# gvanhoy/gr-liquiddsp

Measured on AMD Instinct MI355X. Metric: Msamples/s through flex_rx (QPSK r1/2 1024B), higher is better.
Workload: dtype f32; 1 GPU; flex_rx single stream per GPU, 20000000 samples (10 Msym), PSK4 r=1/2 (CONV_V27), 1024-B payload, CRC-24, 256-sample gaps, CFO/phase/delay + AWGN Es/N0=20 dB; frames_decoded_ok=1154, streams_per_gpu=1, blocks_in_flight=12, stage_events=none (fxrx_set_timing level 0), steps=1415, passes=independent captures (reset between passes), segments=256, repairs=0

## Files before the change

gr-liquiddsp_amd/csrc/fx_kernels.hip:

```cpp
#include <hip/hip_runtime.h>
#include <algorithm>
#include "fx_device.h"
#include "fx_launch.h"
#include "fx_vbclean.h"
#include "fx_rsgmd.h"

#define HALF         256

template <int WW> struct WalkLdsT {
    static constexpr int WAVES = WW;
    static constexpr bool SWEEP_PAIRS = WW == 4;
    float2 win[FX_NFFT];
    float2 X[FX_NFFT];
    float2 S[FX_NFFT];
    float2 scr[WW][576];
    float2 v[640];
    float2 P[256];
    float  m2[FX_NFFT];
    float2 hdr[FX_HDR_SYM];
    float2 cw[(WW + 1) * FX_HOP + 8];
    __device__ __forceinline__ float2 *scr2(int wave) { return wave < 2 ? v + 576 * wave : cw + 576 * (wave - 2); }
    float2 pb[16];
    float2 eqw[16];
    float  taps[FX_MF_TAPS];
// ... 1677 lines not shown
#undef FX_CHAIN_LAUNCH
    return hipGetLastError();
}

template <bool SOFT>
__global__ __launch_bounds__(64 * FX_FLEX_WAVES)
void fx_hdrdec_kernel(const uint8_t *in, uint32_t n, uint8_t *out, int32_t *valid, const FxTables *T)
{
    __shared__ WalkLdsT<FX_FLEX_WAVES> L;
    const int tid = threadIdx.x;
    for (uint32_t h = blockIdx.x; h < n; h += gridDim.x) {
        if constexpr (SOFT) { for (int i = tid; i < 8 * FX_HDR_ENC; i += 64 * FX_FLEX_WAVES) L.hsoft()[i] = in[(size_t)h * (8 * FX_HDR_ENC) + i]; }
        else if (tid < FX_HDR_ENC) L.b0[tid] = in[(size_t)h * FX_HDR_ENC + tid];
        __syncthreads();
        if constexpr (SOFT) decode_header_soft(L, T, tid); else decode_header_bytes(L, T, tid);
        if (tid < FX_HDR_DEC) out[(size_t)h * FX_HDR_DEC + tid] = L.b1[tid];
        if (tid == 0) valid[h] = (int32_t)L.u[1];
        __syncthreads();
    }
}
extern "C" hipError_t fx_launch_hdrdec(int soft, unsigned n, hipStream_t st, const uint8_t *in, uint8_t *out, int32_t *valid, const FxTables *T)
{
    if (n == 0) return hipSuccess;
    const unsigned grid = std::min(n, 65536u);
    if (soft) hipLaunchKernelGGL((fx_hdrdec_kernel<true>), dim3(grid), dim3(64 * FX_FLEX_WAVES), 0, st, in, n, out, valid, T);
    else hipLaunchKernelGGL((fx_hdrdec_kernel<false>), dim3(grid), dim3(64 * FX_FLEX_WAVES), 0, st, in, n, out, valid, T);
    return hipGetLastError();
}

#define PLAN_THREADS 256
#define PLAN_NV 7
enum { PV_SYM = 0, PV_BYTE, PV_DW, PV_OUT, PV_MF, PV_JOB, PV_VB };

__device__ __forceinline__ unsigned pll_class(unsigned ms)
{
    switch (ms) {
    case FX_MODEM_PSK2: return 0; case FX_MODEM_PSK4: return 1; case FX_MODEM_PSK8: return 2; case FX_MODEM_PSK16: return 3;
    case FX_MODEM_DPSK2: return 4; case FX_MODEM_DPSK4: return 5; case FX_MODEM_DPSK8: return 6; case FX_MODEM_ASK4: return 7;
    case FX_MODEM_QAM16: return 8; case FX_MODEM_QAM32: return 9; case FX_MODEM_QAM64: return 10; default: return 11;
    }
}

template <int NT> __device__ __forceinline__ void plan_scan(uint32_t (&v)[PLAN_NV], uint32_t (&tot)[PLAN_NV], uint32_t (*ws)[PLAN_NV])
{
    const int tid = threadIdx.x, lane = tid & 63, wave = tid >> 6;
    uint32_t inc[PLAN_NV];
#pragma unroll
    for (int q = 0; q < PLAN_NV; q++) {
        inc[q] = v[q];
#pragma unroll
        for (int d = 1; d < 64; d <<= 1) { const uint32_t o = (uint32_t)__shfl_up((int)inc[q], d, 64); if (lane >= d) inc[q] += o; }
    }
    __syncthreads();
    if (lane == 63) for (int q = 0; q < PLAN_NV; q++) ws[wave][q] = inc[q];
    __syncthreads();
#pragma unroll
    for (int q = 0; q < PLAN_NV; q++) {
        uint32_t wb = 0, t = 0;
#pragma unroll
        for (int w = 0; w < NT / 64; w++) { const uint32_t x = ws[w][q]; if (w < wave) wb += x; t += x; }
        tot[q] = t; v[q] = wb + inc[q] - v[q];
    }
}

#define PLAN_MAXG 256
enum { PW_TICKET = 0, PW_CLS_CNT = 16, PW_DEC_CNT = 28, PW_VBC_CNT = 31, PW_CLS_FILL = 38, PW_DEC_FILL = 50, PW_VBC_FILL = 53,
       PW_FLAG = 128, PW_AGG = 384, PW_INC = 384 + 8 * PLAN_MAXG, PW_WORDS = 384 + 16 * PLAN_MAXG };

__device__ __forceinline__ uint32_t wave_agg_add(uint32_t *counters, uint32_t key, uint32_t inc, bool active)
{
    const int lane = threadIdx.x & 63;
    unsigned long long rem = __ballot(active);
    uint32_t result = 0;
    while (rem) {
        const int leader = __ffsll((long long)rem) - 1;
        const uint32_t k = (uint32_t)__shfl((int)key, leader, 64);
        const bool mine = active && key == k;
        const unsigned long long same = __ballot(mine);
        uint32_t incl = mine ? inc : 0u;
#pragma unroll
        for (int d = 1; d < 64; d <<= 1) { const uint32_t o = (uint32_t)__shfl_up((int)incl, d, 64); if (lane >= d) incl += o; }
        const uint32_t total = (uint32_t)__shfl((int)incl, 63, 64);
        uint32_t base = 0;
        if (lane == leader) base = atomicAdd(&counters[k], total);
        base = (uint32_t)__shfl((int)base, leader, 64);
        if (mine) result = base + incl - inc;
        rem &= ~same;
    }
    return result;
}

struct PlanWords { uint32_t flags, nsym, plen, ms, check, fec0, fec1; };
__device__ __forceinline__ PlanWords plan_words(const FxFrame *fp) { return { fp->flags, fp->pay_sym_len, fp->pay_len, fp->ms, fp->check, fp->fec0, fp->fec1 }; }
struct PlanFrame {
    const FxFrame *fp = nullptr; uint32_t sidx = 0, bps = 0, k = 0, l0 = 0, l1 = 0, nblk = 0, vnb = 0; bool valid = false, batch = false;
};
__device__ __forceinline__ PlanFrame plan_sizes(const PlanWords &w, bool live, uint32_t detect, uint32_t vb_blk, uint32_t (&v)[PLAN_NV])
{
    PlanFrame f;
#pragma unroll
    for (int q = 0; q < PLAN_NV; q++) v[q] = 0u;
    f.valid = live && !detect && (w.flags & FX_FLAG_HEADER_VALID);
    if (!f.valid) return f;
    f.bps = modem_bps(w.ms);
    f.k = w.plen + crc_len(w.check); f.l0 = fec_enc_len(w.fec0, f.k); f.l1 = fec_enc_len(w.fec1, f.l0);
    f.nblk = (w.nsym + 1023u) / 1024u;
    v[PV_SYM] = (w.nsym + 7u) & ~7u;
    v[PV_BYTE] = (max(f.l1, f.k) + 8u + 15u) & ~15u;
    v[PV_DW] = ((8u * max(f.l0, f.k) + 6u + 63u) & ~63u) + 64u;
    v[PV_OUT] = (w.plen + 15u) & ~15u;
    v[PV_MF] = f.nblk; v[PV_JOB] = 1u;
    f.batch = vb_blk && conv_p(w.fec0) && !conv_p(w.fec1) && w.fec1 != FX_FEC_RS_M8;
    if (f.batch) { f.vnb = (8u * f.k + 6u + vb_blk - 1u) / vb_blk; v[PV_VB] = f.vnb; }
    return f;
}
__device__ __forceinline__ bool plan_demote(uint32_t vb_before, uint32_t vnb, uint32_t vb_cap) { return (uint64_t)vb_before + vnb + 7u * 128u > vb_cap; }

struct PlanKey {
    uint32_t cls, rs, vc;
    __device__ uint32_t dec(bool batch) const { return batch ? 2u : rs; }
    __device__ uint32_t pack() const { return cls | rs << 4 | vc << 5; }
    __device__ static PlanKey unpack(uint32_t p) { return { p & 15u, (p >> 4) & 1u, (p >> 5) & 7u }; }
};
__device__ __forceinline__ PlanKey plan_key(uint32_t ms, uint32_t fec0, uint32_t fec1)
{
    const uint32_t p = (uint32_t)conv_p(fec0);
    return { pll_class(ms), (fec0 == FX_FEC_RS_M8 || fec1 == FX_FEC_RS_M8) ? 1u : 0u, p ? p - 1u : 0u };
}

__device__ __forceinline__ uint32_t plan_stream_of(const uint32_t *base, uint32_t nstreams, uint32_t g)
{
    uint32_t lo = 0, hi = nstreams;
    while (hi - lo > 1) { const uint32_t mid = (lo + hi) >> 1; if (base[mid] <= g) lo = mid; else hi = mid; }
    return lo;
}

struct PlanRest {
    const float2 *x, *xa_end; int64_t abs_base;
    int64_t start; int32_t offset; float rxy, tau, gamma, dphi, phi; uint32_t pfb; int32_t mfc0; uint32_t mix_th, mix_dl; float mf_scale;
    float pilot_dphi, pilot_phi, pilot_gain; uint32_t pll_th; float pll_f; uint32_t header[FX_HDR_DEC / 4];
};
__device__ __forceinline__ PlanRest plan_rest(const FxFrame *__restrict__ fp, const FxStreamDesc *__restrict__ sd)
{
    PlanRest r;
    r.x = sd->x; r.xa_end = sd->xa_end; r.abs_base = sd->abs_base;
    r.start = fp->start; r.offset = fp->offset; r.rxy = fp->rxy; r.tau = fp->tau; r.gamma = fp->gamma; r.dphi = fp->dphi; r.phi = fp->phi;
    r.pfb = fp->pfb; r.mfc0 = fp->mfc0; r.mix_th = fp->mix_th; r.mix_dl = fp->mix_dl; r.mf_scale = fp->mf_scale;
    r.pilot_dphi = fp->pilot_dphi; r.pilot_phi = fp->pilot_phi; r.pilot_gain = fp->pilot_gain; r.pll_th = fp->pll_th; r.pll_f = fp->pll_f;
    const uint32_t *hw = reinterpret_cast<const uint32_t *>(fp->header);
#pragma unroll
    for (int i = 0; i < FX_HDR_DEC / 4; i++) r.header[i] = hw[i];
    return r;
}
__device__ __forceinline__ void plan_emit(FxPayJob *__restrict__ job, FxOutRec *__restrict__ rec, const PlanRest &fp,
                                          const PlanWords &w, const PlanFrame &f, const uint32_t (&off)[PLAN_NV], uint32_t eq, uint32_t slot, uint32_t vb_off)
{
    FxPayJob j;
    j.x = fp.x; j.xa_end = fp.xa_end; j.start = fp.start; j.mix_th = fp.mix_th; j.mix_dl = fp.mix_dl; j.mf_scale = fp.mf_scale;
    j.pfb = fp.pfb; j.mfc0 = fp.mfc0; j.pll_th = fp.pll_th; j.pll_f = fp.pll_f; j.ms = w.ms; j.bps = f.bps;
    j.nsym = f.valid ? w.nsym : 0u; j.sym_off = off[PV_SYM];
    j.pay_len = w.plen; j.check = w.check; j.fec0 = w.fec0; j.fec1 = w.fec1; j.k = f.k; j.l0 = f.l0; j.l1 = f.l1;
    j.byte_off = off[PV_BYTE]; j.dw_off = off[PV_DW]; j.out_off = off[PV_OUT]; j.pad_ = f.valid ? 1u : 0u;
    j.eq = eq; j.chain_idx = slot; j.vb_off = vb_off; j.vb_nblk = (uint16_t)f.vnb; j.vb_clean = 0;
    *job = j;
    union { FxOutRec r; uint4 q[sizeof(FxOutRec) / 16]; } u;
    u.r.start = fp.abs_base + fp.start; u.r.stream = f.sidx; u.r.offset = fp.offset;
    u.r.rxy = fp.rxy; u.r.tau = fp.tau; u.r.gamma = fp.gamma; u.r.dphi = fp.dphi; u.r.phi = fp.phi; u.r.pfb = fp.pfb;
    u.r.pilot_dphi = fp.pilot_dphi; u.r.pilot_phi = fp.pilot_phi; u.r.pilot_gain = fp.pilot_gain;
    u.r.flags = w.flags & FX_FLAG_HEADER_VALID;
    u.r.pay_len = f.valid ? w.plen : 0u; u.r.ms = w.ms; u.r.check = w.check; u.r.fec0 = w.fec0; u.r.fec1 = w.fec1;
    u.r.nsym = f.valid ? w.nsym : 0u; u.r.bps = f.bps; u.r.sym_off = off[PV_SYM]; u.r.out_off = off[PV_OUT];
    u.r.evm_sum = 0.0f; u.r.payload_valid = 0; u.r.status = 0;
    uint32_t *rw = reinterpret_cast<uint32_t *>(u.r.header);
#pragma unroll
    for (int i = 0; i < FX_HDR_DEC / 4; i++) rw[i] = fp.header[i];
    u.r.byte_off = off[PV_BYTE];
    uint4 *dst = reinterpret_cast<uint4 *>(rec);
#pragma unroll
    for (int i = 0; i < (int)(sizeof(FxOutRec) / 16); i++) dst[i] = u.q[i];
}

template <bool AGENT> struct PlanCounts {
    const uint32_t *cls_, *dec_, *vbc_;
    __device__ __forceinline__ static uint32_t ld(const uint32_t *p)
    {
        if constexpr (AGENT) return __hip_atomic_load(p, __ATOMIC_RELAXED, __HIP_MEMORY_SCOPE_AGENT); else return *p;
    }
    __device__ __forceinline__ uint32_t cls(int c) const { return ld(cls_ + c); }
    __device__ __forceinline__ uint32_t dec(int c) const { return ld(dec_ + c); }
    __device__ __forceinline__ uint32_t vbc(int c) const { return ld(vbc_ + c); }
};
template <class Counts> __device__ __forceinline__ void plan_class_bases(const Counts &cnt, uint32_t (&cls_base)[FX_PLL_CLASSES + 1], uint32_t (&vbc_base)[8])
{
    uint32_t b = 0;
    for (int c = 0; c < FX_PLL_CLASSES; c++) { cls_base[c] = b; b += (cnt.cls(c) + 63u) & ~63u; }
    cls_base[FX_PLL_CLASSES] = b;
    uint32_t vb = 0;
    for (int c = 0; c < 7; c++) { vbc_base[c] = vb; vb += (cnt.vbc(c) + 127u) & ~127u; }
    vbc_base[7] = vb;
}
template <int NT, class Counts> __device__ __forceinline__ void plan_pad_lists(const Counts &cnt, const uint32_t (&cls_base)[FX_PLL_CLASSES + 1], const uint32_t (&vbc_base)[8], const FxPlanArgs &a)
{
    for (int c = 0; c < FX_PLL_CLASSES; c++)
        for (uint32_t i = cls_base[c] + cnt.cls(c) + threadIdx.x; i < cls_base[c + 1] && i < a.list_cap; i += NT) a.pll_list[i] = 0xFFFFFFFFu;
    for (int c = 0; c < 7; c++)
        for (uint32_t i = vbc_base[c] + cnt.vbc(c) + threadIdx.x; i < vbc_base[c + 1] && i < a.vb_cap; i += NT) a.vb_items[i] = 0xFFFFFFFFu;
}
template <class Tot, class Counts> __device__ __forceinline__ void plan_fill_hdr(FxBlockHdr &h, uint32_t N, Tot tot, const Counts &cnt, const uint32_t (&cls_base)[FX_PLL_CLASSES + 1],
                                                                                 const uint32_t (&vbc_base)[8], const FxPlanArgs &a)
{
    h.n_frames = N; h.n_pjobs = tot[PV_JOB]; h.n_mfblk = min(tot[PV_MF], a.mf_cap);
    h.n_dec_plain = cnt.dec(0); h.n_dec_rs = cnt.dec(1); h.n_dec_batch = cnt.dec(2);
    h.n_vb_items = min(vbc_base[7], a.vb_cap); h.vb_blk = a.vb_blk; h.vb_want = tot[PV_VB] + 7u * 128u; h.n_vb_fallback = 0;
    for (int c = 0; c < FX_PLL_CLASSES; c++) { h.pll_cnt[c] = cnt.cls(c); h.pll_base[c] = cls_base[c]; }
    h.pll_base[FX_PLL_CLASSES] = cls_base[FX_PLL_CLASSES];
    h.sym_total = tot[PV_SYM]; h.byte_total = tot[PV_BYTE]; h.dw_total = tot[PV_DW]; h.out_total = tot[PV_OUT];
    h.done = 1;
}
template <int NT> __device__ __forceinline__ void plan_mirror_hdr(const FxBlockHdr &h, const FxPlanArgs &a)
{
    const uint32_t *src = reinterpret_cast<const uint32_t *>(&h);
    uint32_t *d0 = reinterpret_cast<uint32_t *>(a.hdr_pay), *d1 = reinterpret_cast<uint32_t *>(a.hdr_host), *z = reinterpret_cast<uint32_t *>(a.hdr);
    for (int i = threadIdx.x; i < (int)(sizeof(FxBlockHdr) / 4); i += NT) { const uint32_t w = src[i]; d0[i] = w; d1[i] = w; z[i] = 0u; }
}

__device__ __forceinline__ PlanFrame plan_frame(uint32_t g, bool live, const FxPlanArgs &a, PlanWords &w, uint32_t (&v)[PLAN_NV])
{
    const uint32_t sidx = live ? plan_stream_of(a.stream_base, a.nstreams, g) : 0u;
    const FxFrame *fp = live ? a.chain + a.streams[sidx].chain_base + (g - a.stream_base[sidx]) : nullptr;
    w = live ? plan_words(fp) : PlanWords{};
    PlanFrame f = plan_sizes(w, live, a.detect, a.vb_blk, v);
    f.fp = fp; f.sidx = sidx;
    return f;
}
__device__ __forceinline__ void plan_range(uint32_t N, uint32_t &g0, uint32_t &g1)
{
    const uint32_t per = ((N + gridDim.x - 1) / gridDim.x + PLAN_THREADS - 1) / PLAN_THREADS * PLAN_THREADS;
    g0 = min(N, blockIdx.x * per); g1 = min(N, g0 + per);
}
template <int NT> __device__ __forceinline__ uint32_t plan_stream_bases(const uint32_t *chain_count, uint32_t nstreams, uint32_t *stream_base, uint32_t (*ws)[PLAN_NV])
{
    const int tid = threadIdx.x;
    uint32_t run = 0;
    for (uint32_t s0 = 0; s0 < nstreams; s0 += NT) {
        const uint32_t sidx = s0 + tid;
        uint32_t v[PLAN_NV] = { sidx < nstreams ? chain_count[sidx] : 0u, 0, 0, 0, 0, 0, 0 }, tot[PLAN_NV];
        plan_scan<NT>(v, tot, ws);
        if (sidx < nstreams) stream_base[sidx] = run + v[0];
        run += tot[0];
        __syncthreads();
    }
    if (tid == 0) stream_base[nstreams] = run;
    __threadfence(); __syncthreads(); __threadfence();
    return run;
}

extern "C" __global__ __launch_bounds__(PLAN_THREADS)
void fx_plan_kernel(const FxPlanArgs a)
{
    __shared__ uint32_t ws[PLAN_THREADS / 64][PLAN_NV];
    __shared__ uint32_t base_s[PLAN_NV];
    uint32_t *const pw = a.ws;
    const int tid = threadIdx.x;
    const uint32_t N = plan_stream_bases<PLAN_THREADS>(a.chain_count, a.nstreams, a.stream_base, ws);
    uint32_t g0, g1; plan_range(N, g0, g1);
    const uint32_t wg = blockIdx.x;
    uint32_t run[PLAN_NV] = { 0, 0, 0, 0, 0, 0, 0 };
    for (uint32_t c0 = g0; c0 < g1; c0 += PLAN_THREADS) {
        uint32_t v[PLAN_NV], tot[PLAN_NV]; PlanWords w;
        (void)plan_frame(c0 + tid, c0 + tid < g1, a, w, v);
        plan_scan<PLAN_THREADS>(v, tot, ws);
#pragma unroll
        for (int q = 0; q < PLAN_NV; q++) run[q] += tot[q];
        __syncthreads();
    }
    if (tid == 0) {
        uint32_t base[PLAN_NV] = { 0, 0, 0, 0, 0, 0, 0 };
        if (wg > 0) {
            for (int q = 0; q < PLAN_NV; q++) pw[PW_AGG + 8 * wg + q] = run[q];
            __threadfence();
            __hip_atomic_store(&pw[PW_FLAG + wg], 1u, __ATOMIC_RELEASE, __HIP_MEMORY_SCOPE_AGENT);
            for (int p = (int)wg - 1; p >= 0; p--) {
                uint32_t f;
                do { f = __hip_atomic_load(&pw[PW_FLAG + p], __ATOMIC_ACQUIRE, __HIP_MEMORY_SCOPE_AGENT); if (!f) __builtin_amdgcn_s_sleep(2); } while (!f);
                const volatile uint32_t *src = pw + (f == 2u ? PW_INC : PW_AGG) + 8 * p;
                for (int q = 0; q < PLAN_NV; q++) base[q] += src[q];
                if (f == 2u) break;
            }
        }
        for (int q = 0; q < PLAN_NV; q++) { pw[PW_INC + 8 * wg + q] = base[q] + run[q]; base_s[q] = base[q]; }
        __threadfence();
        __hip_atomic_store(&pw[PW_FLAG + wg], 2u, __ATOMIC_RELEASE, __HIP_MEMORY_SCOPE_AGENT);
    }
    __syncthreads();
    uint32_t before[PLAN_NV];
#pragma unroll
    for (int q = 0; q < PLAN_NV; q++) before[q] = base_s[q];
    for (uint32_t c0 = g0; c0 < g1; c0 += PLAN_THREADS) {
        const uint32_t g = c0 + tid;
        const bool live = g < g1;
        uint32_t v[PLAN_NV], tot[PLAN_NV]; PlanWords w;
        PlanFrame f = plan_frame(g, live, a, w, v);
        plan_scan<PLAN_THREADS>(v, tot, ws);
#pragma unroll
        for (int q = 0; q < PLAN_NV; q++) { v[q] += before[q]; before[q] += tot[q]; }
        if (f.batch && plan_demote(v[PV_VB], f.vnb, a.vb_cap)) { f.batch = false; f.vnb = 0; }
        if (live) {
            plan_emit(a.pjobs + g, a.recs + g, plan_rest(f.fp, a.streams + f.sidx), w, f, v, a.eq, (uint32_t)(f.fp - a.chain), 0u);
            for (uint32_t c = 0; c < f.nblk; c++) if (v[PV_MF] + c < a.mf_cap) { a.mf_job[v[PV_MF] + c] = g; a.mf_c0[v[PV_MF] + c] = c * 1024u; }
        }
        {
            const PlanKey key = plan_key(w.ms, w.fec0, w.fec1);
            (void)wave_agg_add(pw + PW_CLS_CNT, key.cls, 1u, f.valid);
            (void)wave_agg_add(pw + PW_DEC_CNT, key.dec(f.batch), 1u, f.valid);
            (void)wave_agg_add(pw + PW_VBC_CNT, key.vc, f.vnb, f.batch);
        }
        __syncthreads();
    }
}

extern "C" __global__ __launch_bounds__(PLAN_THREADS)
void fx_planlists_kernel(const FxPlanArgs a)
{
    __shared__ struct { FxBlockHdr h; uint32_t cls_base[FX_PLL_CLASSES + 1], vbc_base[8], last; } sh;
    uint32_t *const pw = a.ws;
    const PlanCounts<true> cnt{ pw + PW_CLS_CNT, pw + PW_DEC_CNT, pw + PW_VBC_CNT };
    const int tid = threadIdx.x;
    const uint32_t N = __hip_atomic_load(&a.stream_base[a.nstreams], __ATOMIC_RELAXED, __HIP_MEMORY_SCOPE_AGENT);
    if (tid == 0) plan_class_bases(cnt, sh.cls_base, sh.vbc_base);
    __syncthreads();
    uint32_t g0, g1; plan_range(N, g0, g1);
    for (uint32_t c0 = g0; c0 < g1; c0 += PLAN_THREADS) {
        const uint32_t g = c0 + tid;
        const bool live = g < g1;
        uint32_t ms = 0, fec0 = 0, fec1 = 0, vnb = 0; bool val = false;
        if (live) { const FxPayJob &j = a.pjobs[g]; val = j.pad_ != 0; ms = j.ms; fec0 = j.fec0; fec1 = j.fec1; vnb = j.vb_nblk; }
        const PlanKey key = plan_key(ms, fec0, fec1);
        const bool bt = val && vnb;
        const uint32_t pp = sh.cls_base[key.cls] + wave_agg_add(pw + PW_CLS_FILL, key.cls, 1u, val);
        if (val && pp < a.list_cap) a.pll_list[pp] = g;
        const uint32_t rs = key.dec(bt), dp = wave_agg_add(pw + PW_DEC_FILL, rs, 1u, val);
        if (val && dp < a.list_cap) a.dec_list[(size_t)rs * a.list_cap + dp] = g;
        const uint32_t at = sh.vbc_base[key.vc] + wave_agg_add(pw + PW_VBC_FILL, key.vc, vnb, bt);
        if (bt) a.pjobs[g].vb_off = at;
    }
    if (blockIdx.x == 0) plan_pad_lists<PLAN_THREADS>(cnt, sh.cls_base, sh.vbc_base, a);
    __threadfence(); __syncthreads();
    if (tid == 0) sh.last = atomicAdd(&pw[PW_TICKET], 1u) == gridDim.x - 1 ? 1u : 0u;
    __syncthreads();
    if (!sh.last) return;
    __threadfence();
    if (tid == 0) {
        sh.h = *a.hdr;
        plan_fill_hdr(sh.h, N, (const volatile uint32_t *)(pw + PW_INC + 8 * (gridDim.x - 1)), cnt, sh.cls_base, sh.vbc_base, a);
    }
    __syncthreads();
    plan_mirror_hdr<PLAN_THREADS>(sh.h, a);
    for (int i = tid; i < PW_WORDS; i += PLAN_THREADS) pw[i] = 0u;
}

#define PLAN_TILE 2048
#define PLAN_BATCH 2
#define PLAN_LDS_STREAMS 256
enum { PO_CLS = 0, PO_DEC = FX_PLL_CLASSES, PO_VBC = FX_PLL_CLASSES + 4, PO_N = FX_PLL_CLASSES + 12 };
template <int NT> struct PlanOneShared {
    FxBlockHdr h;
    uint32_t ws[NT / 64][PLAN_NV];
    uint32_t cnt[PO_N], fill[PO_N];
    uint32_t cls_base[FX_PLL_CLASSES + 1], vbc_base[8];
    uint32_t sbase[PLAN_LDS_STREAMS + 1], cbase[PLAN_LDS_STREAMS];
};
template <int NT> __device__ __forceinline__ uint32_t plan_one_slot(uint32_t g, const FxPlanArgs &a, const PlanOneShared<NT> &sh, uint32_t &sidx)
{
    if (a.nstreams <= PLAN_LDS_STREAMS) { sidx = plan_stream_of(sh.sbase, a.nstreams, g); return sh.cbase[sidx] + (g - sh.sbase[sidx]); }
    sidx = plan_stream_of(a.stream_base, a.nstreams, g);
    return a.streams[sidx].chain_base + (g - a.stream_base[sidx]);
}

template <int NT> __global__ __launch_bounds__(NT)
void fx_planfused_kernel(const FxPlanArgs a)
{
    constexpr uint32_t TILE = PLAN_TILE;
    constexpr int KEEP = PLAN_TILE / NT, JB = PLAN_BATCH;
    static_assert(NT % 64 == 0 && KEEP * NT == PLAN_TILE && KEEP % JB == 0, "whole waves; the tile is KEEP frames a thread, in whole batches");
    __shared__ PlanOneShared<NT> sh;
    __shared__ uint2 keep[PLAN_TILE];
    const PlanCounts<false> cnt{ sh.cnt + PO_CLS, sh.cnt + PO_DEC, sh.cnt + PO_VBC };
    const uint32_t tid = threadIdx.x, nstreams = a.nstreams;
#ifdef FX_STAMPS
    unsigned long long tk_ = __builtin_readcyclecounter(); uint32_t st1_ = 0, st2_ = 0, st6_ = 0, st7_ = 0;
#define PLAN_TICK(acc) do { const unsigned long long t_ = __builtin_readcyclecounter(); acc += (uint32_t)(t_ - tk_); tk_ = t_; } while (0)
#else
#define PLAN_TICK(acc) do { } while (0)
#endif
    {
        const uint32_t *src = reinterpret_cast<const uint32_t *>(a.hdr); uint32_t *dst = reinterpret_cast<uint32_t *>(&sh.h);
        for (int i = (int)tid; i < (int)(sizeof(FxBlockHdr) / 4); i += NT) dst[i] = src[i];
        if (tid < PO_N) { sh.cnt[tid] = 0u; sh.fill[tid] = 0u; }
        if (tid <= FX_PLL_CLASSES) sh.cls_base[tid] = 0u;
        if (tid < 8) sh.vbc_base[tid] = 0u;
    }
    uint32_t N;
    if (nstreams <= PLAN_LDS_STREAMS) {
        uint32_t v[PLAN_NV] = { tid < nstreams ? a.chain_count[tid] : 0u, 0, 0, 0, 0, 0, 0 }, tot[PLAN_NV];
        if (nstreams > 1) plan_scan<NT>(v, tot, sh.ws); else { tot[0] = v[0]; v[0] = 0u; }
        if (tid < nstreams) { sh.sbase[tid] = v[0]; a.stream_base[tid] = v[0]; sh.cbase[tid] = a.streams[tid].chain_base; }
        if (tid == 0) { sh.sbase[nstreams] = tot[0]; a.stream_base[nstreams] = tot[0]; }
        __syncthreads();
        N = sh.sbase[nstreams];
    } else N = plan_stream_bases<NT>(a.chain_count, nstreams, a.stream_base, sh.ws);

    uint32_t run[PLAN_NV] = { 0, 0, 0, 0, 0, 0, 0 };
    for (int pass = N > TILE ? 0 : 1; pass < 2; pass++) {
#pragma unroll
        for (int q = 0; q < PLAN_NV; q++) run[q] = 0u;
        for (uint32_t t0 = 0; t0 < N; t0 += TILE) {
            const uint32_t nt = min(TILE, N - t0), t1 = t0 + nt, per = (nt + NT - 1) / NT, f0 = t0 + tid * per;
            uint32_t st[PLAN_NV];
            PlanWords w[KEEP]; uint32_t slot[KEEP], sidx[KEEP];
#pragma unroll
            for (int i = 0; i < KEEP; i++) {
                const bool live = (uint32_t)i < per && f0 + i < t1;
                slot[i] = plan_one_slot(live ? f0 + i : t0, a, sh, sidx[i]);
                w[i] = plan_words(a.chain + slot[i]);
            }
#pragma unroll
            for (int q = 0; q < PLAN_NV; q++) st[q] = 0u;
#pragma unroll
            for (int i = 0; i < KEEP; i++) {
                uint32_t v[PLAN_NV];
                (void)plan_sizes(w[i], (uint32_t)i < per && f0 + i < t1, a.detect, a.vb_blk, v);
#pragma unroll
                for (int q = 0; q < PLAN_NV; q++) st[q] += v[q];
            }
            {
                uint32_t tot[PLAN_NV];
                plan_scan<NT>(st, tot, sh.ws);
#pragma unroll
                for (int q = 0; q < PLAN_NV; q++) { st[q] += run[q]; run[q] += tot[q]; }
            }
            if (pass == 0 || N <= TILE) {
                uint32_t vb = st[PV_VB];
#pragma unroll
                for (int i = 0; i < KEEP; i++) {
                    uint32_t v[PLAN_NV];
                    const PlanFrame f = plan_sizes(w[i], (uint32_t)i < per && f0 + i < t1, a.detect, a.vb_blk, v);
                    const bool batch = f.batch && !plan_demote(vb, f.vnb, a.vb_cap);
                    vb += f.vnb;
                    if (f.valid) {
                        const PlanKey key = plan_key(w[i].ms, w[i].fec0, w[i].fec1);
                        atomicAdd(&sh.cnt[PO_CLS + key.cls], 1u);
                        atomicAdd(&sh.cnt[PO_DEC + key.dec(batch)], 1u);
                        if (batch) atomicAdd(&sh.cnt[PO_VBC + key.vc], f.vnb);
                    }
                }
            }
            if (pass == 0) continue;
            if (t0 == 0) {
                __syncthreads();
                if (tid == 0) plan_class_bases(cnt, sh.cls_base, sh.vbc_base);
                __syncthreads();
            }
            PLAN_TICK(st1_);
#pragma unroll
            for (int b0 = 0; b0 < KEEP; b0 += JB) {
                if ((uint32_t)b0 >= per) break;
                PlanRest r[JB];
#pragma unroll
                for (int i = 0; i < JB; i++) r[i] = plan_rest(a.chain + slot[b0 + i], a.streams + sidx[b0 + i]);
#pragma unroll
                for (int i = 0; i < JB; i++) {
                    const uint32_t g = f0 + b0 + i;
                    if ((uint32_t)(b0 + i) >= per || g >= t1) break;
                    const PlanWords &wi = w[b0 + i];
                    uint32_t v[PLAN_NV];
                    PlanFrame f = plan_sizes(wi, true, a.detect, a.vb_blk, v);
                    f.fp = a.chain + slot[b0 + i]; f.sidx = sidx[b0 + i];
                    if (f.batch && plan_demote(st[PV_VB], f.vnb, a.vb_cap)) { f.batch = false; f.vnb = 0; }
                    uint32_t at = 0;
                    if (f.valid) {
                        const PlanKey key = plan_key(wi.ms, wi.fec0, wi.fec1);
                        const uint32_t pp = sh.cls_base[key.cls] + atomicAdd(&sh.fill[PO_CLS + key.cls], 1u);
                        if (pp < a.list_cap) a.pll_list[pp] = g;
                        const uint32_t rs = key.dec(f.batch), dp = atomicAdd(&sh.fill[PO_DEC + rs], 1u);
                        if (dp < a.list_cap) a.dec_list[(size_t)rs * a.list_cap + dp] = g;
                        if (f.batch) at = sh.vbc_base[key.vc] + atomicAdd(&sh.fill[PO_VBC + key.vc], f.vnb);
                    }
                    keep[g - t0] = make_uint2(st[PV_MF], f.nblk);
                    plan_emit(a.pjobs + g, a.recs + g, r[i], wi, f, st, a.eq, slot[b0 + i], at);
#pragma unroll
                    for (int q = 0; q < PLAN_NV; q++) st[q] += v[q];
                }
            }
            __syncthreads();
            PLAN_TICK(st2_);
            for (uint32_t k = tid >> 4; k < nt; k += NT / 16) {
                const uint2 kp = keep[k];
                const uint32_t g = t0 + k, sub = tid & 15u;
                for (uint32_t c = sub; c < kp.y; c += 16u) if (kp.x + c < a.mf_cap) { a.mf_job[kp.x + c] = g; a.mf_c0[kp.x + c] = c * 1024u; }
            }
            __syncthreads();
        }
    }
    plan_pad_lists<NT>(cnt, sh.cls_base, sh.vbc_base, a);
    PLAN_TICK(st6_);
    __threadfence(); __syncthreads();
    PLAN_TICK(st7_);
    if (tid == 0) {
#ifdef FX_STAMPS
        sh.h.stamp[1] = st1_; sh.h.stamp[2] = st2_; sh.h.stamp[6] = st6_; sh.h.stamp[7] = st7_;
#endif
        plan_fill_hdr(sh.h, N, run, cnt, sh.cls_base, sh.vbc_base, a);
    }
    __syncthreads();
    plan_mirror_hdr<NT>(sh.h, a);
}

extern "C" hipError_t fx_launch_plan(hipStream_t st, unsigned grid, int fused, unsigned threads, const FxPlanArgs &a)
{
    const unsigned g = grid < 1u ? 1u : (grid > PLAN_MAXG ? PLAN_MAXG : grid);
    if (fused && g == 1u) {
        if (threads == 512u) hipLaunchKernelGGL((fx_planfused_kernel<512>), dim3(1), dim3(512), 0, st, a);
        else if (threads == 256u) hipLaunchKernelGGL((fx_planfused_kernel<256>), dim3(1), dim3(256), 0, st, a);
        else return hipErrorInvalidValue;
    } else {
        hipLaunchKernelGGL(fx_plan_kernel, dim3(g), dim3(PLAN_THREADS), 0, st, a);
        hipLaunchKernelGGL(fx_planlists_kernel, dim3(g), dim3(PLAN_THREADS), 0, st, a);
    }
    return hipGetLastError();
}
extern "C" unsigned fx_plan_ws_words(void) { return PW_WORDS; }

#define PMF_THREADS 256
#define PMF_SYMS    1024
#define PMF_SPAN    (2 * PMF_SYMS + FX_MF_TAPS)

__global__ __launch_bounds__(PMF_THREADS)
void fx_paymf_kernel(const FxPayJob *jobs, const uint32_t *blk_job, const uint32_t *blk_c0, const FxBlockHdr *hdr, const FxFrame *chain, float2 *sym_raw,
                     const FxTables *T)
{
    constexpr int LEAD = FX_EQ_TAPS - 1;
    __shared__ float2 v[PMF_SPAN + LEAD + 4];
    __shared__ float2 u[2 * PMF_SYMS + FX_EQ_TAPS];
    __shared__ float2 eqw[16];
    __shared__ float taps[FX_MF_TAPS];
    const uint32_t nitems = hdr->n_mfblk;
    const int tid = threadIdx.x;
    const float2 *sc = T->sc;
    for (uint32_t bi = blockIdx.x; bi < nitems; bi += gridDim.x) {
        const FxPayJob job = jobs[blk_job[bi]];
        const uint32_t c0 = blk_c0[bi];
        const uint32_t ns = min((uint32_t)PMF_SYMS, job.nsym - c0);
        const int64_t sym0 = (int64_t)FX_SYM0_PAY + FX_EQ_DELAY;
        const int64_t nlo = sym_sample(sym0 + c0, job.mfc0) - LEAD - (FX_MF_TAPS - 1);
        const int64_t nhi = sym_sample(sym0 + c0 + ns - 1, job.mfc0);
        const int span = (int)(nhi - nlo + 1);
        const XSrc xs = make_xsrc(job.x, job.xa_end, 0);
        __syncthreads();
        if (tid < FX_MF_TAPS) taps[tid] = T->proto[job.pfb + FX_NPFB * tid];
        if (tid < 16) eqw[tid] = tid < FX_EQ_TAPS ? chain[job.chain_idx].eq[tid] : make_float2(0.0f, 0.0f);
        for (int m = tid; m < span; m += PMF_THREADS) {
            const int64_t nn = nlo + m;
            v[m] = derot(xld(xs, job.start + nn), job.mix_th + job.mix_dl * (uint32_t)nn, sc);
        }
        __syncthreads();
        const int nu = span - (FX_MF_TAPS - 1);
        for (int m = tid; m < nu; m += PMF_THREADS) {
            const float2 y = mf_sum<7>(v, taps, m + (FX_MF_TAPS - 1));
            u[m] = make_float2(y.x * job.mf_scale, y.y * job.mf_scale);
        }
        __syncthreads();
        for (uint32_t i = tid; i < ns; i += PMF_THREADS) {
            const int nc = (int)(sym_sample(sym0 + c0 + i, job.mfc0) - nlo) - (FX_MF_TAPS - 1);
            sym_raw[(size_t)job.sym_off + c0 + i] = eq_sum16(u + nc - (FX_EQ_TAPS - 1), eqw);
        }
    }
}

#define PMF4_STRIDE 274
extern "C" __global__ __launch_bounds__(PMF_THREADS)
void fx_paymf4_kernel(const FxPayJob *jobs, const uint32_t *blk_job, const uint32_t *blk_c0, const FxBlockHdr *hdr, float2 *sym_raw, const FxTables *T)
{
    __shared__ float2 ph[8 * PMF4_STRIDE];
    __shared__ __attribute__((aligned(16))) float taps[FX_MF_TAPS];
    static_assert(FX_MF_TAPS == 28 && PMF_SYMS == 4 * PMF_THREADS, "tile below: 28 taps, four symbols per thread");
    static_assert(PMF4_STRIDE >= (PMF_SPAN + 8) / 8 + 5, "phase arrays hold the span plus the slack phantom symbols read");
    const uint32_t nitems = hdr->n_mfblk;
    const int tid = threadIdx.x;
    const float2 *sc = T->sc;
    for (uint32_t bi = blockIdx.x; bi < nitems; bi += gridDim.x) {
        const FxPayJob job = jobs[blk_job[bi]];
        const uint32_t c0 = blk_c0[bi];
        const uint32_t ns = min((uint32_t)PMF_SYMS, job.nsym - c0);
        const int64_t nlo = sym_sample((int64_t)FX_SYM0_PAY + c0, job.mfc0) - (FX_MF_TAPS - 1);
        const int span = 2 * (int)ns + (FX_MF_TAPS - 2);
        const float2 *px = job.x, *pa = job.xa_end;
        const int64_t p0 = job.start + nlo;
        const uint32_t th0 = job.mix_th + job.mix_dl * (uint32_t)nlo, dl = job.mix_dl;
        __syncthreads();
        if (tid < FX_MF_TAPS) taps[tid] = T->proto[job.pfb + FX_NPFB * tid];
        constexpr int NLD = (PMF_SPAN + PMF_THREADS - 1) / PMF_THREADS;
        float2 raw[NLD];
#pragma unroll
        for (int k = 0; k < NLD; k++) {
            const int m = tid + PMF_THREADS * k;
            const int64_t p = p0 + m;
            raw[k] = m < span ? (p < 0 ? pa[p] : px[p]) : make_float2(0.0f, 0.0f);
        }
#pragma unroll
        for (int k = 0; k < NLD; k++) {
            const int m = tid + PMF_THREADS * k;
            const int j = m >> 1;
            if (m < span) ph[((m & 1) * 4 + (j & 3)) * PMF4_STRIDE + (j >> 2)] = derot(raw[k], th0 + dl * (uint32_t)m, sc);
        }
        __syncthreads();
        if (4u * (uint32_t)tid < ns) {
            float2 e[17], o[17];
#pragma unroll
            for (int j = 0; j < 17; j++) {
                e[j] = ph[(j & 3) * PMF4_STRIDE + tid + (j >> 2)];
                o[j] = ph[(4 + (j & 3)) * PMF4_STRIDE + tid + (j >> 2)];
            }
            float h[FX_MF_TAPS];
#pragma unroll
            for (int q = 0; q < FX_MF_TAPS / 4; q++) { const float4 t4 = reinterpret_cast<const float4 *>(taps)[q]; h[4 * q] = t4.x; h[4 * q + 1] = t4.y; h[4 * q + 2] = t4.z; h[4 * q + 3] = t4.w; }
            float yr[4], yi[4];
#pragma unroll
            for (int r = 0; r < 4; r++) {
                float ar = 0.0f, ai = 0.0f;
#pragma unroll
                for (int k = 0; k < 14; k++) {
                    ar = fmaf(h[2 * k], o[13 + r - k].x, ar); ai = fmaf(h[2 * k], o[13 + r - k].y, ai);
                    ar = fmaf(h[2 * k + 1], e[13 + r - k].x, ar); ai = fmaf(h[2 * k + 1], e[13 + r - k].y, ai);
                }
                yr[r] = ar * job.mf_scale; yi[r] = ai * job.mf_scale;
            }
            float4 *dst = reinterpret_cast<float4 *>(sym_raw + (size_t)job.sym_off + c0 + 4u * (uint32_t)tid);
            dst[0] = make_float4(yr[0], yi[0], yr[1], yi[1]);
            dst[1] = make_float4(yr[2], yi[2], yr[3], yi[3]);
        }
    }
}

extern "C" hipError_t fx_launch_paymf(unsigned grid, int eq, hipStream_t st, const FxPayJob *jobs, const uint32_t *blk_job, const uint32_t *blk_c0, const FxBlockHdr *hdr,
                                      const FxFrame *chain, float2 *sym_raw, const FxTables *T)
{
    if (grid == 0) return hipSuccess;
    if (eq) hipLaunchKernelGGL(fx_paymf_kernel, dim3(grid), dim3(PMF_THREADS), 0, st, jobs, blk_job, blk_c0, hdr, chain, sym_raw, T);
    else hipLaunchKernelGGL(fx_paymf4_kernel, dim3(grid), dim3(PMF_THREADS), 0, st, jobs, blk_job, blk_c0, hdr, sym_raw, T);
    return hipGetLastError();
}

#define PLL_THREADS 64
#define PLL_MAX_WAVES 4
#define PLL_BLK     8
#define PLL_AHEAD   3
#define PLL_RING    (PLL_AHEAD + 1)

__device__ __forceinline__ void pll_load8(const float4 *p, float4 b[4]) { b[0] = p[0]; b[1] = p[1]; b[2] = p[2]; b[3] = p[3]; }

template <int MS>
__device__ __forceinline__ unsigned pll_demod(float2 r, unsigned &prev, const float2 *sc, float2 &xh, float &pe)
{
// ... 2254 lines not shown
```

Baseline: 46860 Msamples/s.

## Stage plan job and record writes through LDS for coalesced stores

In the fused planner kernel, each thread used to write its 128-byte FxPayJob and FxOutRec straight to global memory. Because consecutive frames of a thread are strided by `per`, those stores were scattered. Each wave now puts its per-lane structs into a padded LDS staging buffer, orders with wavefront fences and barriers, then cooperatively writes them out so eight lanes cover one 128-byte struct as uint4s. This adds LDS traffic, wave barriers and a ballot per frame, and dead lanes now run plan_sizes with have=false instead of exiting early.

Result: no change. 47230 Msamples/s, median of 6 (+0.8%).

```diff
diff --git a/gr-liquiddsp_amd/csrc/fx_kernels.hip b/gr-liquiddsp_amd/csrc/fx_kernels.hip
--- a/gr-liquiddsp_amd/csrc/fx_kernels.hip
+++ b/gr-liquiddsp_amd/csrc/fx_kernels.hip
@@ -1853,8 +1853,9 @@
     for (int i = 0; i < FX_HDR_DEC / 4; i++) r.header[i] = hw[i];
     return r;
 }
-__device__ __forceinline__ void plan_emit(FxPayJob *__restrict__ job, FxOutRec *__restrict__ rec, const PlanRest &fp,
-                                          const PlanWords &w, const PlanFrame &f, const uint32_t (&off)[PLAN_NV], uint32_t eq, uint32_t slot, uint32_t vb_off)
+template <class T> union PlanPieces { T v; uint4 q[8]; static_assert(sizeof(T) == 8 * sizeof(uint4), "a job or a record: 128 bytes"); };
+__device__ __forceinline__ FxPayJob plan_job(const PlanRest &fp, const PlanWords &w, const PlanFrame &f, const uint32_t (&off)[PLAN_NV],
+                                             uint32_t eq, uint32_t slot, uint32_t vb_off)
 {
     FxPayJob j;
     j.x = fp.x; j.xa_end = fp.xa_end; j.start = fp.start; j.mix_th = fp.mix_th; j.mix_dl = fp.mix_dl; j.mf_scale = fp.mf_scale;
@@ -1863,22 +1864,59 @@
     j.pay_len = w.plen; j.check = w.check; j.fec0 = w.fec0; j.fec1 = w.fec1; j.k = f.k; j.l0 = f.l0; j.l1 = f.l1;
     j.byte_off = off[PV_BYTE]; j.dw_off = off[PV_DW]; j.out_off = off[PV_OUT]; j.pad_ = f.valid ? 1u : 0u;
     j.eq = eq; j.chain_idx = slot; j.vb_off = vb_off; j.vb_nblk = (uint16_t)f.vnb; j.vb_clean = 0;
-    *job = j;
-    union { FxOutRec r; uint4 q[sizeof(FxOutRec) / 16]; } u;
-    u.r.start = fp.abs_base + fp.start; u.r.stream = f.sidx; u.r.offset = fp.offset;
-    u.r.rxy = fp.rxy; u.r.tau = fp.tau; u.r.gamma = fp.gamma; u.r.dphi = fp.dphi; u.r.phi = fp.phi; u.r.pfb = fp.pfb;
-    u.r.pilot_dphi = fp.pilot_dphi; u.r.pilot_phi = fp.pilot_phi; u.r.pilot_gain = fp.pilot_gain;
-    u.r.flags = w.flags & FX_FLAG_HEADER_VALID;
-    u.r.pay_len = f.valid ? w.plen : 0u; u.r.ms = w.ms; u.r.check = w.check; u.r.fec0 = w.fec0; u.r.fec1 = w.fec1;
-    u.r.nsym = f.valid ? w.nsym : 0u; u.r.bps = f.bps; u.r.sym_off = off[PV_SYM]; u.r.out_off = off[PV_OUT];
-    u.r.evm_sum = 0.0f; u.r.payload_valid = 0; u.r.status = 0;
-    uint32_t *rw = reinterpret_cast<uint32_t *>(u.r.header);
+    return j;
+}
+__device__ __forceinline__ FxOutRec plan_rec(const PlanRest &fp, const PlanWords &w, const PlanFrame &f, const uint32_t (&off)[PLAN_NV])
+{
+    FxOutRec r;
+    r.start = fp.abs_base + fp.start; r.stream = f.sidx; r.offset = fp.offset;
+    r.rxy = fp.rxy; r.tau = fp.tau; r.gamma = fp.gamma; r.dphi = fp.dphi; r.phi = fp.phi; r.pfb = fp.pfb;
+    r.pilot_dphi = fp.pilot_dphi; r.pilot_phi = fp.pilot_phi; r.pilot_gain = fp.pilot_gain;
+    r.flags = w.flags & FX_FLAG_HEADER_VALID;
+    r.pay_len = f.valid ? w.plen : 0u; r.ms = w.ms; r.check = w.check; r.fec0 = w.fec0; r.fec1 = w.fec1;
+    r.nsym = f.valid ? w.nsym : 0u; r.bps = f.bps; r.sym_off = off[PV_SYM]; r.out_off = off[PV_OUT];
+    r.evm_sum = 0.0f; r.payload_valid = 0; r.status = 0;
+    uint32_t *rw = reinterpret_cast<uint32_t *>(r.header);
 #pragma unroll
     for (int i = 0; i < FX_HDR_DEC / 4; i++) rw[i] = fp.header[i];
-    u.r.byte_off = off[PV_BYTE];
+    r.byte_off = off[PV_BYTE];
+    return r;
+}
+__device__ __forceinline__ void plan_emit(FxPayJob *__restrict__ job, FxOutRec *__restrict__ rec, const PlanRest &fp,
+                                          const PlanWords &w, const PlanFrame &f, const uint32_t (&off)[PLAN_NV], uint32_t eq, uint32_t slot, uint32_t vb_off)
+{
+    *job = plan_job(fp, w, f, off, eq, slot, vb_off);
+    PlanPieces<FxOutRec> u; u.v = plan_rec(fp, w, f, off);
     uint4 *dst = reinterpret_cast<uint4 *>(rec);
 #pragma unroll
-    for (int i = 0; i < (int)(sizeof(FxOutRec) / 16); i++) dst[i] = u.q[i];
+    for (int i = 0; i < 8; i++) dst[i] = u.q[i];
+}
+#define PLAN_STAGE_ROW 9u
+__device__ __forceinline__ uint32_t plan_stage_at(uint32_t r, uint32_t p) { return r * PLAN_STAGE_ROW + p; }
+__device__ __forceinline__ void plan_wave_order()
+{
+    __builtin_amdgcn_fence(__ATOMIC_RELEASE, "wavefront"); __builtin_amdgcn_wave_barrier(); __builtin_amdgcn_fence(__ATOMIC_ACQUIRE, "wavefront");
+}
+template <class T> __device__ __forceinline__ void plan_stage_put(uint4 *stage, uint32_t lane, const T &v)
+{
+    PlanPieces<T> u; u.v = v;
+#pragma unroll
+    for (uint32_t p = 0; p < 8u; p++) stage[plan_stage_at(lane, p)] = u.q[p];
+}
+template <class T> __device__ __forceinline__ void plan_stage_out(const uint4 *stage, uint32_t lane, uint32_t nlive, T *__restrict__ dst0, uint32_t stride)
+{
+    const uint32_t p = lane & 7u;
+#pragma unroll
+    for (uint32_t j0 = 0; j0 < 8u; j0 += 4u) {
+        uint4 q[4];
+#pragma unroll
+        for (uint32_t j = 0; j < 4u; j++) q[j] = stage[plan_stage_at((lane >> 3) + 8u * (j0 + j), p)];
+#pragma unroll
+        for (uint32_t j = 0; j < 4u; j++) {
+            const uint32_t r = (lane >> 3) + 8u * (j0 + j);
+            if (r < nlive) reinterpret_cast<uint4 *>(dst0 + (size_t)r * stride)[p] = q[j];
+        }
+    }
 }
 
 template <bool AGENT> struct PlanCounts {
@@ -2086,10 +2124,12 @@
     static_assert(NT % 64 == 0 && KEEP * NT == PLAN_TILE && KEEP % JB == 0, "whole waves; the tile is KEEP frames a thread, in whole batches");
     __shared__ PlanOneShared<NT> sh;
     __shared__ uint2 keep[PLAN_TILE];
+    __shared__ uint4 stage[NT / 64][64 * PLAN_STAGE_ROW];
     const PlanCounts<false> cnt{ sh.cnt + PO_CLS, sh.cnt + PO_DEC, sh.cnt + PO_VBC };
-    const uint32_t tid = threadIdx.x, nstreams = a.nstreams;
+    const uint32_t tid = threadIdx.x, lane = tid & 63u, nstreams = a.nstreams;
+    uint4 *const stg = stage[tid >> 6];
 #ifdef FX_STAMPS
-    unsigned long long tk_ = __builtin_readcyclecounter(); uint32_t st1_ = 0, st2_ = 0, st6_ = 0, st7_ = 0;
+    unsigned long long tk_ = __builtin_readcyclecounter(); uint32_t st1_ = 0, st4_ = 0, st5_ = 0, st6_ = 0, st7_ = 0;
 #define PLAN_TICK(acc) do { const unsigned long long t_ = __builtin_readcyclecounter(); acc += (uint32_t)(t_ - tk_); tk_ = t_; } while (0)
 #else
 #define PLAN_TICK(acc) do { } while (0)
@@ -2171,11 +2211,13 @@
                 for (int i = 0; i < JB; i++) r[i] = plan_rest(a.chain + slot[b0 + i], a.streams + sidx[b0 + i]);
 #pragma unroll
                 for (int i = 0; i < JB; i++) {
-                    const uint32_t g = f0 + b0 + i;
-                    if ((uint32_t)(b0 + i) >= per || g >= t1) break;
+                    const uint32_t g = f0 + b0 + i, gw = t0 + (tid - lane) * per + b0 + i;
+                    const bool have = (uint32_t)(b0 + i) < per && g < t1;
+                    const uint32_t nlive = (uint32_t)__popcll(__ballot(have));
+                    if (!nlive) break;
                     const PlanWords &wi = w[b0 + i];
                     uint32_t v[PLAN_NV];
-                    PlanFrame f = plan_sizes(wi, true, a.detect, a.vb_blk, v);
+                    PlanFrame f = plan_sizes(wi, have, a.detect, a.vb_blk, v);
                     f.fp = a.chain + slot[b0 + i]; f.sidx = sidx[b0 + i];
                     if (f.batch && plan_demote(st[PV_VB], f.vnb, a.vb_cap)) { f.batch = false; f.vnb = 0; }
                     uint32_t at = 0;
@@ -2187,14 +2229,27 @@
                         if (dp < a.list_cap) a.dec_list[(size_t)rs * a.list_cap + dp] = g;
                         if (f.batch) at = sh.vbc_base[key.vc] + atomicAdd(&sh.fill[PO_VBC + key.vc], f.vnb);
                     }
-                    keep[g - t0] = make_uint2(st[PV_MF], f.nblk);
-                    plan_emit(a.pjobs + g, a.recs + g, r[i], wi, f, st, a.eq, slot[b0 + i], at);
+                    if (have) keep[g - t0] = make_uint2(st[PV_MF], f.nblk);
+                    const FxPayJob jb = plan_job(r[i], wi, f, st, a.eq, slot[b0 + i], at);
+                    PLAN_TICK(st4_);
+                    plan_stage_put(stg, lane, jb);
+                    plan_wave_order();
+                    plan_stage_out(stg, lane, nlive, a.pjobs + gw, per);
+                    plan_wave_order();
+                    PLAN_TICK(st5_);
+                    const FxOutRec rc = plan_rec(r[i], wi, f, st);
+                    PLAN_TICK(st4_);
+                    plan_stage_put(stg, lane, rc);
+                    plan_wave_order();
+                    plan_stage_out(stg, lane, nlive, a.recs + gw, per);
+                    plan_wave_order();
+                    PLAN_TICK(st5_);
 #pragma unroll
                     for (int q = 0; q < PLAN_NV; q++) st[q] += v[q];
                 }
             }
             __syncthreads();
-            PLAN_TICK(st2_);
+            PLAN_TICK(st4_);
             for (uint32_t k = tid >> 4; k < nt; k += NT / 16) {
                 const uint2 kp = keep[k];
                 const uint32_t g = t0 + k, sub = tid & 15u;
@@ -2209,7 +2264,7 @@
     PLAN_TICK(st7_);
     if (tid == 0) {
 #ifdef FX_STAMPS
-        sh.h.stamp[1] = st1_; sh.h.stamp[2] = st2_; sh.h.stamp[6] = st6_; sh.h.stamp[7] = st7_;
+        sh.h.stamp[1] = st1_; sh.h.stamp[2] = st4_ + st5_; sh.h.stamp[4] = st4_; sh.h.stamp[5] = st5_; sh.h.stamp[6] = st6_; sh.h.stamp[7] = st7_;
 #endif
         plan_fill_hdr(sh.h, N, run, cnt, sh.cls_base, sh.vbc_base, a);
     }
```
